# transferia/transferia

Measured on NVIDIA H100. Metric: ChangeItems/sec on ClickBench-shaped 99-col batches (filter_rows + cast + ClickHouse native block + LZ4 frames), higher is better.
Workload: dtype u8

## Files before the change

transferia_b200/csrc/kernels_encode.cuh:

```cuda
#pragma once
#include "device_types.cuh"

namespace tfk {

__device__ __forceinline__ uint32_t warp_incl_scan(uint32_t v) {
    const unsigned lane = threadIdx.x & 31;
#pragma unroll
    for (int d = 1; d < 32; d <<= 1) { uint32_t t = __shfl_up_sync(0xffffffffu, v, d); if (lane >= (unsigned)d) v += t; }
    return v;
}
__device__ __forceinline__ uint32_t block_excl_scan(uint32_t v, uint32_t* total, uint32_t* smem33) {
    const unsigned lane = threadIdx.x & 31, warp = threadIdx.x >> 5, nw = (blockDim.x + 31) >> 5;
    uint32_t inc = warp_incl_scan(v);
    if (lane == 31) smem33[warp] = inc;
    __syncthreads();
    if (warp == 0) {
        uint32_t w = lane < nw ? smem33[lane] : 0;
        uint32_t wi = warp_incl_scan(w);
        smem33[lane] = wi - w;
        if (lane == 31) smem33[32] = wi;
    }
    __syncthreads();
    uint32_t res = inc - v + smem33[warp];
    *total = smem33[32];
    __syncthreads();
    return res;
}

struct StrictCol { const uint8_t* src; uint8_t* dst; const uint8_t* validity; int32_t src_tf, dst_tf, col, pad; };
struct StrictArgs { const StrictCol* cols; int ncols; uint64_t nrows; uint8_t* err; uint16_t* term; };
__device__ __forceinline__ int64_t go_f2i64(double f) { return (f >= -9223372036854775808.0 && f < 9223372036854775808.0) ? (int64_t)f : INT64_MIN; }
__device__ __forceinline__ uint64_t go_f2u64(double f) { return f < 9223372036854775808.0 ? (uint64_t)go_f2i64(f) : ((uint64_t)go_f2i64(f - 9223372036854775808.0) ^ 0x8000000000000000ull); }
__global__ void k_strictify(StrictArgs a);
#ifdef TF_KERNELS_ENCODE
__global__ void __launch_bounds__(256) k_strictify(StrictArgs a) {
    const uint64_t r = (uint64_t)blockIdx.x * blockDim.x + threadIdx.x;
    if (r >= a.nrows) return;
    int err = 0, term = 0xff;
    for (int k = 0; k < a.ncols; k++) {
        const StrictCol c = a.cols[k];
        if (c.validity && !((c.validity[r >> 3] >> (r & 7)) & 1)) continue;
        int cls; int64_t si = 0; uint64_t ui = 0; double f = 0;
        switch (c.src_tf) {
        case TF_INT8: cls = 0; si = ((const int8_t*)c.src)[r]; break;
        case TF_INT16: cls = 0; si = ((const int16_t*)c.src)[r]; break;
        case TF_INT32: cls = 0; si = ((const int32_t*)c.src)[r]; break;
        case TF_INT64: cls = 0; si = ((const int64_t*)c.src)[r]; break;
        case TF_UINT8: cls = 1; ui = c.src[r]; break;
        case TF_UINT16: cls = 1; ui = ((const uint16_t*)c.src)[r]; break;
        case TF_UINT32: cls = 1; ui = ((const uint32_t*)c.src)[r]; break;
        case TF_UINT64: cls = 1; ui = ((const uint64_t*)c.src)[r]; break;
        case TF_FLOAT: cls = 2; f = ((const float*)c.src)[r]; break;
        case TF_DOUBLE: cls = 2; f = ((const double*)c.src)[r]; break;
        default: cls = 3; si = c.src[r] ? 1 : 0; break;
        }
        int e = 0;
        const int64_t as_i = cls == 0 || cls == 3 ? si : (cls == 1 ? (int64_t)ui : go_f2i64(f));
        const bool neg = cls == 0 ? si < 0 : (cls == 2 ? f < 0 : false);
        const uint64_t as_u = cls == 0 || cls == 3 ? (uint64_t)si : (cls == 1 ? ui : go_f2u64(f));
        auto sint = [&](int64_t lo, int64_t hi) { if (as_i < lo || as_i > hi) e = TF_ROWERR_STRICT_RANGE; };
        auto uint_ = [&](uint64_t hi) { if (neg) e = TF_ROWERR_STRICT_CAST; else if (as_u > hi) e = TF_ROWERR_STRICT_RANGE; };
        switch (c.dst_tf) {
        case TF_INT8: sint(INT8_MIN, INT8_MAX); ((int8_t*)c.dst)[r] = (int8_t)as_i; break;
        case TF_INT16: sint(INT16_MIN, INT16_MAX); ((int16_t*)c.dst)[r] = (int16_t)as_i; break;
        case TF_INT32: sint(INT32_MIN, INT32_MAX); ((int32_t*)c.dst)[r] = (int32_t)as_i; break;
        case TF_INT64: case TF_INTERVAL: case TF_DATE: case TF_DATETIME: case TF_TIMESTAMP:
            ((int64_t*)c.dst)[r] = as_i; break;
        case TF_UINT8: uint_(UINT8_MAX); c.dst[r] = (uint8_t)as_u; break;
        case TF_UINT16: uint_(UINT16_MAX); ((uint16_t*)c.dst)[r] = (uint16_t)as_u; break;
        case TF_UINT32: uint_(UINT32_MAX); ((uint32_t*)c.dst)[r] = (uint32_t)as_u; break;
        case TF_UINT64: uint_(UINT64_MAX); ((uint64_t*)c.dst)[r] = as_u; break;
        case TF_FLOAT: ((float*)c.dst)[r] = cls == 0 || cls == 3 ? (float)si : (cls == 1 ? (float)ui : (float)f); break;
        case TF_DOUBLE: ((double*)c.dst)[r] = cls == 0 ? (double)si : (cls == 1 ? (double)ui : f); break;
        default: c.dst[r] = cls == 2 ? (f != 0) : (cls == 1 ? ui != 0 : si != 0); break;
        }
        if (e && !err) { err = e; term = c.col; }
    }
    const bool mine = err && !a.err[r];
    if (mine) a.err[r] = (uint8_t)err;
    a.term[r] = (uint16_t)(mine ? term : 0xff);
}
#endif

struct RowVal {
    int cls;
    int64_t i; double f; const uint8_t* s; uint32_t slen; uint32_t nsec;
};

__device__ __forceinline__ bool row_valid(const DCol& c, uint64_t r) { return !c.validity || ((c.validity[r >> 3] >> (r & 7)) & 1); }

__device__ __forceinline__ RowVal load_val(const DCol& c, uint64_t r) {
    RowVal v; v.cls = 0; v.i = 0; v.f = 0; v.s = nullptr; v.slen = 0; v.nsec = 0;
    if (!row_valid(c, r)) return v;
    switch (c.type) {
    case TF_INT8:  v.cls = 1; v.i = ((const int8_t*)c.values)[r]; break;
    case TF_INT16: v.cls = 1; v.i = ((const int16_t*)c.values)[r]; break;
    case TF_INT32: v.cls = 1; v.i = ((const int32_t*)c.values)[r]; break;
    case TF_INT64: v.cls = 1; v.i = ((const int64_t*)c.values)[r]; break;
    case TF_UINT8:  v.cls = 1; v.i = ((const uint8_t*)c.values)[r]; break;
    case TF_UINT16: v.cls = 1; v.i = ((const uint16_t*)c.values)[r]; break;
    case TF_UINT32: v.cls = 1; v.i = ((const uint32_t*)c.values)[r]; break;
    case TF_UINT64: { uint64_t u = ((const uint64_t*)c.values)[r]; if (u > 0x7fffffffffffffffULL) v.cls = 8; else { v.cls = 1; v.i = (int64_t)u; } break; }
    case TF_FLOAT:  v.cls = 2; v.f = ((const float*)c.values)[r]; break;
    case TF_DOUBLE: v.cls = 2; v.f = ((const double*)c.values)[r]; break;
    case TF_BOOLEAN: v.cls = 3; v.i = c.values[r] != 0; v.f = v.i ? 1.0 : 0.0; break;
    case TF_INTERVAL: v.cls = 7; break;
    case TF_DATE: case TF_DATETIME: case TF_TIMESTAMP:
        v.cls = 6; v.i = ((const int64_t*)c.values)[r]; v.nsec = c.aux ? ((const uint32_t*)c.aux)[r] : 0; break;
    case TF_BYTES: v.cls = 5; v.s = c.heap + c.offsets[r]; v.slen = c.offsets[r + 1] - c.offsets[r]; break;
    case TF_UTF8:  v.cls = 4; v.s = c.heap + c.offsets[r]; v.slen = c.offsets[r + 1] - c.offsets[r]; break;
    case TF_ANY:
        if (c.aux && c.aux[r] == 1) { v.cls = 4; v.s = c.heap + c.offsets[r]; v.slen = c.offsets[r + 1] - c.offsets[r]; }
        else v.cls = 7;
        break;
    }
    return v;
}

template <typename T> __device__ __forceinline__ bool ordered(T a, T b, int op) {
    switch (op) { case 0: return a == b; case 1: return a != b; case 2: return a < b; case 3: return a <= b; case 4: return a > b; default: return a >= b; }
}
__device__ __forceinline__ int cmp_bytes(const uint8_t* a, uint32_t an, const uint8_t* b, uint32_t bn) {
    uint32_t m = an < bn ? an : bn;
    for (uint32_t k = 0; k < m; k++) { int d = (int)a[k] - (int)b[k]; if (d) return d < 0 ? -1 : 1; }
    return an < bn ? -1 : (an > bn ? 1 : 0);
}
__device__ __forceinline__ bool contains_bytes(const uint8_t* h, uint32_t hn, const uint8_t* n, uint32_t nn) {
    if (nn == 0) return true;
    if (nn > hn) return false;
    const uint8_t n0 = n[0];
    for (uint32_t i = 0; i + nn <= hn; i++) {
        if (h[i] != n0) continue;
        uint32_t k = 1; while (k < nn && h[i + k] == n[k]) k++;
        if (k == nn) return true;
    }
    return false;
}

static __device__ int eval_term(const RowVal& v, const DTerm& t, const uint8_t* blob, bool& matched) {
    const int op = t.op; const bool is_set = (op == 6 || op == 7);
    const int base = t.vtype & 15; const bool is_list = (t.vtype & 16) != 0;
    if (v.cls == 8) return TF_ROWERR_FILTER_OVERFLOW;
    if (op >= 8 && base != 4) return TF_ROWERR_FILTER_TYPEPAIR;
    const bool is_int1 = v.cls == 1;
    const bool is_float1 = v.cls == 2 || v.cls == 3 || v.cls == 0;
    const double float1 = v.cls == 2 ? v.f : (v.cls == 3 ? v.f : 0.0);
    const int64_t* il = (const int64_t*)(blob + t.list_off);
    const double* fl = (const double*)(blob + t.list_off);
    switch (base) {
    case 1:
        if (is_int1) {
            if (is_set) { bool c = false; for (int k = 0; k < t.nlist; k++) c |= (il[k] == v.i); matched = (op == 6) ? c : !c; return 0; }
            matched = ordered<int64_t>(v.i, t.i, op); return 0;
// ... 134 lines not shown
}
#endif

__global__ void k_compact_sel(const uint8_t* keep, const uint32_t* blockoff, uint64_t nrows, uint32_t* sel);
#ifdef TF_KERNELS_ENCODE
__global__ void __launch_bounds__(256) k_compact_sel(const uint8_t* keep, const uint32_t* blockoff, uint64_t nrows, uint32_t* sel) {
    __shared__ uint32_t sm[33];
    const uint64_t r = (uint64_t)blockIdx.x * blockDim.x + threadIdx.x;
    const uint32_t k = (r < nrows && keep[r]) ? 1u : 0u;
    uint32_t tot; const uint32_t ex = block_excl_scan(k, &tot, sm);
    if (k) sel[blockoff[blockIdx.x] + ex] = (uint32_t)r;
}
#endif

struct LayoutArgs {
    DCol* cols; int ncols;
    const int32_t* out_cols;
    const int32_t* str_cols; int nstr;
    const uint32_t* tile_sum;
    uint64_t* tile_base;
    uint32_t ntiles_cap;
    const uint8_t* col_headers; const uint32_t* col_header_off;
    uint8_t* raw; DState* st;
    uint64_t nrows_in; int has_sel; uint32_t frame_bytes;
    uint64_t* col_bytes;
};

#define TF_STR_TILE 256
#define TF_STR_THREADS 256
#define TF_STR_STAGE 16384

__global__ void k_layout_scan(LayoutArgs a);
#ifdef TF_KERNELS_ENCODE
__global__ void __launch_bounds__(1024) k_layout_scan(LayoutArgs a) {
    __shared__ uint32_t sm[33];
    const int s = blockIdx.x;
    const uint64_t n = a.st->n_kept;
    const uint32_t ntiles = (uint32_t)((n + TF_STR_TILE - 1) / TF_STR_TILE);
    uint64_t carry = 0;
    for (uint32_t base = 0; base < ntiles; base += blockDim.x) {
        const uint32_t i = base + threadIdx.x;
        const uint32_t v = i < ntiles ? a.tile_sum[(size_t)s * a.ntiles_cap + i] : 0;
        uint32_t tot; const uint32_t ex = block_excl_scan(v, &tot, sm);
        if (i < ntiles) a.tile_base[(size_t)s * a.ntiles_cap + i] = carry + ex;
        carry += tot;
    }
    if (threadIdx.x == 0) a.col_bytes[s] = carry;
}
#endif

__global__ void k_layout_finish(LayoutArgs a);
#ifdef TF_KERNELS_ENCODE
__global__ void __launch_bounds__(256) k_layout_finish(LayoutArgs a) {
    __shared__ uint64_t s_size[3][256];
    __shared__ uint64_t s_pos[256];
    __shared__ uint64_t s_run;
    const uint64_t n = a.st->n_kept;
    if (threadIdx.x == 0) {
        uint8_t* o = a.raw; uint64_t p = 0;
        o[p++] = 1; o[p++] = 0; o[p++] = 2; o[p++] = 0xff; o[p++] = 0xff; o[p++] = 0xff; o[p++] = 0xff; o[p++] = 0;
        uint64_t v = (uint64_t)a.ncols; while (v >= 0x80) { o[p++] = (uint8_t)(v | 0x80); v >>= 7; } o[p++] = (uint8_t)v;
        v = n; while (v >= 0x80) { o[p++] = (uint8_t)(v | 0x80); v >>= 7; } o[p++] = (uint8_t)v;
        s_run = p;
    }
    for (int base = 0; base < a.ncols; base += 256) {
        const int c = base + threadIdx.x;
        __syncthreads();
        if (c < a.ncols) {
            const DCol& d = a.cols[a.out_cols[c]];
            s_size[0][threadIdx.x] = a.col_header_off[c + 1] - a.col_header_off[c];
            s_size[1][threadIdx.x] = (d.nullable && n) ? n : 0;
            s_size[2][threadIdx.x] = n ? ((d.out_kind == OK_STR || d.out_kind == OK_TOSTR) ? a.col_bytes[d.str_slot] : (uint64_t)d.out_w * n) : 0;
        }
        __syncthreads();
        if (threadIdx.x == 0) {
            uint64_t p = s_run; const int m = a.ncols - base < 256 ? a.ncols - base : 256;
            for (int k = 0; k < m; k++) { s_pos[k] = p; p += s_size[0][k] + s_size[1][k] + s_size[2][k]; }
            s_run = p;
        }
        __syncthreads();
        if (c < a.ncols) {
            DCol& d = a.cols[a.out_cols[c]];
            const uint64_t p = s_pos[threadIdx.x];
            d.hdr_off = p; d.null_off = p + s_size[0][threadIdx.x]; d.out_off = d.null_off + s_size[1][threadIdx.x];
            const uint32_t hb = a.col_header_off[c], hn = (uint32_t)s_size[0][threadIdx.x];
            for (uint32_t k = 0; k < hn; k++) a.raw[p + k] = a.col_headers[hb + k];
        }
    }
    __syncthreads();
    if (threadIdx.x == 0) {
        const uint64_t p = s_run;
        a.st->raw_total = p;
        a.st->n_frames = p ? (p + a.frame_bytes - 1) / a.frame_bytes : 1;
        a.st->frame_ticket = 0;
    }
}
#endif

struct ColRegions { uint64_t values, validity, aux, offsets, heap, heap_len; };

__global__ void k_layout_columnar(LayoutArgs a, ColRegions* regions);
#ifdef TF_KERNELS_ENCODE
__global__ void __launch_bounds__(256) k_layout_columnar(LayoutArgs a, ColRegions* regions) {
    __shared__ uint64_t s_sz[5][256];
    __shared__ uint64_t s_pos[256];
    __shared__ uint64_t s_run;
    const uint64_t n = a.st->n_kept;
    if (threadIdx.x == 0) s_run = 0;
    for (int base = 0; base < a.ncols; base += 256) {
        const int k = base + threadIdx.x;
        __syncthreads();
        if (k < a.ncols) {
            const DCol& d = a.cols[a.out_cols[k]];
            const bool var = d.out_kind == OK_STR || d.out_kind == OK_MASK || d.out_kind == OK_TOSTR;
            const bool fresh = d.out_kind == OK_MASK || d.out_kind == OK_TOSTR || d.out_kind == OK_TODT;
            const uint64_t heap = (d.out_kind == OK_STR || d.out_kind == OK_TOSTR) ? a.col_bytes[d.str_slot] : (d.out_kind == OK_MASK ? 64 * n : 0);
            s_sz[0][threadIdx.x] = var ? 0 : (uint64_t)d.out_w * n;
            s_sz[1][threadIdx.x] = (d.validity && !fresh) ? (n + 7) / 8 : 0;
            s_sz[2][threadIdx.x] = (d.aux && !fresh) ? (d.type == TF_ANY ? n : 4 * n) : 0;
            s_sz[3][threadIdx.x] = var ? 4 * (n + 1) : 0;
            s_sz[4][threadIdx.x] = heap;
        }
        __syncthreads();
        if (threadIdx.x == 0) {
            uint64_t p = s_run; const int m = a.ncols - base < 256 ? a.ncols - base : 256;
            for (int q = 0; q < m; q++) { s_pos[q] = p; for (int z = 0; z < 5; z++) p += (s_sz[z][q] + 15) & ~15ull; }
            s_run = p;
        }
        __syncthreads();
        if (k < a.ncols) {
            DCol& d = a.cols[a.out_cols[k]];
            uint64_t p = s_pos[threadIdx.x]; ColRegions r;
            auto take = [&](int z) { const uint64_t at = p; p += (s_sz[z][threadIdx.x] + 15) & ~15ull; return at; };
            const uint64_t v = take(0), val = take(1), ax = take(2), of = take(3), hp = take(4);
            const bool var = d.out_kind == OK_STR || d.out_kind == OK_MASK || d.out_kind == OK_TOSTR;
            d.out_off = var ? hp : v; d.null_off = val; d.aux_off = ax; d.offs_off = of;
            r.values = var ? ~0ull : v; r.validity = s_sz[1][threadIdx.x] ? val : ~0ull; r.aux = s_sz[2][threadIdx.x] ? ax : ~0ull;
            r.offsets = var ? of : ~0ull; r.heap = var ? hp : ~0ull; r.heap_len = s_sz[4][threadIdx.x];
            regions[k] = r;
            if (var) ((uint32_t*)(a.raw + of))[n] = (uint32_t)s_sz[4][threadIdx.x];
        }
    }
    __syncthreads();
    if (threadIdx.x == 0) { a.st->raw_total = s_run; a.st->n_frames = 0; a.st->frame_ticket = 0; }
}
#endif

struct EncodeArgs {
    const DCol* cols;
    const int32_t* slots;
    const uint32_t* sel; const DState* st; uint8_t* raw;
    uint32_t* tile_sum; const uint64_t* tile_base; uint32_t ntiles_cap;
    int columnar;
};

#define TF_SLOT_NULLMAP (1 << 30)
#define TF_SLOT_AUX (1 << 29)
#define TF_SLOT_ZEROMAP (1 << 28)
#define TF_FIX_TILE_WORDS 2048
#define CH_MAX_DATE_SEC 4291747200LL

enum StreamKind { SK_COPY = 0, SK_BOOL, SK_DATE, SK_DATETIME, SK_TS64, SK_NULLMAP, SK_AUX32, SK_AUX8, SK_ZERO, SK_TODT_CH, SK_TODT_SEC };

template <int K, int INW> __device__ __forceinline__ uint64_t elem_t(const DCol& c, const uint32_t* sel, uint64_t j, uint64_t n) {
    if (j >= n) return 0;
    const uint64_t r = sel ? sel[j] : j;
    if (K == SK_ZERO) return 0;
    if (K == SK_TODT_CH || K == SK_TODT_SEC) {
        int64_t s = 0;
        if (row_valid(c, r)) s = c.type == TF_INT32 ? (int64_t)((const int32_t*)c.values)[r] : (int64_t)((const uint32_t*)c.values)[r];
        if (K == SK_TODT_SEC) return (uint64_t)s;
        if (s > CH_MAX_DATE_SEC) s = CH_MAX_DATE_SEC;
        if (s < 0) s = 0;
        return (uint64_t)s;
    }
    if (K == SK_AUX8) return (uint64_t)c.aux[r];
    if (K == SK_AUX32) return (uint64_t)((const uint32_t*)c.aux)[r];
    const bool valid = row_valid(c, r);
    if (K == SK_NULLMAP) return valid ? 0 : 1;
    if (!valid) return 0;
    if (K == SK_COPY) {
        if (INW == 1) return c.values[r];
        if (INW == 2) return ((const uint16_t*)c.values)[r];
        if (INW == 4) return ((const uint32_t*)c.values)[r];
        return ((const uint64_t*)c.values)[r];
    }
    if (K == SK_BOOL) return c.values[r] != 0;
    if (K == SK_DATE || K == SK_DATETIME) {
        int64_t s = ((const int64_t*)c.values)[r];
        const uint32_t ns = c.aux ? ((const uint32_t*)c.aux)[r] : 0;
        if (s > CH_MAX_DATE_SEC || (s == CH_MAX_DATE_SEC && ns > 0)) s = CH_MAX_DATE_SEC;
        if (s < 0) s = 0;
        return K == SK_DATE ? (uint64_t)(s / 86400) : (uint64_t)s;
    }
    const int64_t s = ((const int64_t*)c.values)[r];
    const uint32_t ns = c.aux ? ((const uint32_t*)c.aux)[r] : 0;
    return (uint64_t)(s * 1000000LL + (int64_t)(ns / 1000u));
}

template <int K, int INW, int W> __device__ __forceinline__ uint32_t stream_word_t(const DCol& c, const uint32_t* sel, uint64_t q, uint64_t n) {
    if (W == 1) return (uint32_t)elem_t<K, INW>(c, sel, 4 * q, n) | ((uint32_t)elem_t<K, INW>(c, sel, 4 * q + 1, n) << 8) |
                       ((uint32_t)elem_t<K, INW>(c, sel, 4 * q + 2, n) << 16) | ((uint32_t)elem_t<K, INW>(c, sel, 4 * q + 3, n) << 24);
    if (W == 2) return (uint32_t)(elem_t<K, INW>(c, sel, 2 * q, n) & 0xffff) | ((uint32_t)(elem_t<K, INW>(c, sel, 2 * q + 1, n) & 0xffff) << 16);
    if (W == 4) return (uint32_t)elem_t<K, INW>(c, sel, q, n);
    const uint64_t v = elem_t<K, INW>(c, sel, q >> 1, n); return (uint32_t)(v >> ((q & 1) * 32));
}

template <int K, int INW, int W> __device__ __forceinline__ void encode_stream(const DCol& c, const EncodeArgs& a, uint64_t base, uint64_t n) {
    const uint32_t m = (uint32_t)(base & 3);
    const uint64_t total = n * (uint64_t)W;
    const uint64_t T = (m + total + 3) >> 2;
    uint8_t* dst0 = a.raw + (base - m);
    const unsigned lane = threadIdx.x & 31;
    for (uint64_t t0 = (uint64_t)blockIdx.x * TF_FIX_TILE_WORDS; t0 < T; t0 += (uint64_t)gridDim.x * TF_FIX_TILE_WORDS)
#pragma unroll 2
    for (uint32_t it = 0; it < TF_FIX_TILE_WORDS / 256; it++) {
        const uint64_t t = t0 + it * 256 + threadIdx.x;
        const uint32_t wcur = (t < T) ? stream_word_t<K, INW, W>(c, a.sel, t, n) : 0;
        uint32_t wprev = __shfl_up_sync(0xffffffffu, wcur, 1);
        if (lane == 0) wprev = (m && t > 0 && t <= T) ? stream_word_t<K, INW, W>(c, a.sel, t - 1, n) : 0;
        if (t >= T) continue;
        const uint32_t val = m ? __funnelshift_r(wprev, wcur, 8 * (4 - m)) : wcur;
        const int64_t sb = (int64_t)(4 * t) - (int64_t)m;
        uint8_t* dst = dst0 + 4 * t;
        if (sb >= 0 && (uint64_t)sb + 4 <= total) *(uint32_t*)dst = val;
        else {
#pragma unroll
            for (int b = 0; b < 4; b++) { const int64_t x = sb + b; if (x >= 0 && (uint64_t)x < total) dst[b] = (uint8_t)(val >> (8 * b)); }
        }
    }
}

__global__ void k_encode_fixed(EncodeArgs a);
#ifdef TF_KERNELS_ENCODE
__global__ void __launch_bounds__(256) k_encode_fixed(EncodeArgs a) {
    const int32_t slot = a.slots[blockIdx.y];
    const DCol c = a.cols[slot & ~(TF_SLOT_NULLMAP | TF_SLOT_AUX | TF_SLOT_ZEROMAP)];
    const uint64_t n = a.st->n_kept;
    if (n == 0) return;
    const DCol& cc = c;
    if (slot & TF_SLOT_ZEROMAP) { encode_stream<SK_ZERO, 1, 1>(cc, a, c.null_off, n); return; }
    if (slot & TF_SLOT_NULLMAP) { encode_stream<SK_NULLMAP, 1, 1>(c, a, c.null_off, n); return; }
    if (slot & TF_SLOT_AUX) { if (c.type == TF_ANY) encode_stream<SK_AUX8, 1, 1>(c, a, c.aux_off, n); else encode_stream<SK_AUX32, 4, 4>(c, a, c.aux_off, n); return; }
    switch (c.out_kind) {
    case OK_COPY:
        switch (c.in_w) {
        case 1: encode_stream<SK_COPY, 1, 1>(c, a, c.out_off, n); break;
        case 2: encode_stream<SK_COPY, 2, 2>(c, a, c.out_off, n); break;
        case 4: encode_stream<SK_COPY, 4, 4>(c, a, c.out_off, n); break;
        default: encode_stream<SK_COPY, 8, 8>(c, a, c.out_off, n); break;
        }
        break;
    case OK_BOOL: encode_stream<SK_BOOL, 1, 1>(c, a, c.out_off, n); break;
    case OK_DATE: encode_stream<SK_DATE, 8, 2>(c, a, c.out_off, n); break;
    case OK_DATETIME: encode_stream<SK_DATETIME, 8, 4>(c, a, c.out_off, n); break;
    case OK_TS64: encode_stream<SK_TS64, 8, 8>(c, a, c.out_off, n); break;
    case OK_TODT: if (a.columnar) encode_stream<SK_TODT_SEC, 4, 8>(c, a, c.out_off, n); else encode_stream<SK_TODT_CH, 4, 4>(c, a, c.out_off, n); break;
    }
}
#endif

__global__ void k_pack_validity(EncodeArgs a);
#ifdef TF_KERNELS_ENCODE
__global__ void __launch_bounds__(256) k_pack_validity(EncodeArgs a) {
    const DCol c = a.cols[a.slots[blockIdx.y]];
    const uint64_t n = a.st->n_kept;
    const uint64_t b = (uint64_t)blockIdx.x * blockDim.x + threadIdx.x;
    if (b * 8 >= n) return;
    uint32_t v = 0;
#pragma unroll
    for (int k = 0; k < 8; k++) {
        const uint64_t j = b * 8 + k;
        if (j < n) { const uint64_t r = a.sel ? a.sel[j] : j; v |= (row_valid(c, r) ? 1u : 0u) << k; }
    }
    a.raw[c.null_off + b] = (uint8_t)v;
}
#endif


struct MeasureArgs { const DCol* cols; int ncols; uint64_t nrows; uint64_t* per_row; unsigned long long* total; };

__global__ void k_measure(MeasureArgs a);
#ifdef TF_KERNELS_ENCODE
__global__ void __launch_bounds__(256) k_measure(MeasureArgs a) {
    __shared__ uint32_t sm[33];
    const uint64_t r = (uint64_t)blockIdx.x * blockDim.x + threadIdx.x;
    uint64_t sz = 0;
    if (r < a.nrows) {
        sz = 24;
        for (int c = 0; c < a.ncols; c++) {
            const DCol& d = a.cols[c];
            sz += 16;
            if (!row_valid(d, r)) continue;
            switch (d.type) {
            case TF_UTF8: sz += 16 + (d.offsets[r + 1] - d.offsets[r]); break;
            case TF_ANY: sz += 16 + (d.offsets[r + 1] - d.offsets[r]); break;
            case TF_BYTES: sz += 24 + (d.offsets[r + 1] - d.offsets[r]); break;
            case TF_DATE: case TF_DATETIME: case TF_TIMESTAMP: sz += 24; break;
            default: sz += (uint64_t)d.in_w;
            }
        }
        if (a.per_row) a.per_row[r] = sz;
    }
    const uint32_t lo = (uint32_t)(sz & 0xffffffu), hi = (uint32_t)(sz >> 24);
    uint32_t tl, th; block_excl_scan(lo, &tl, sm); __syncthreads(); block_excl_scan(hi, &th, sm);
    if (threadIdx.x == 0) atomicAdd(a.total, (unsigned long long)tl + ((unsigned long long)th << 24));
}
#endif

}
```

transferia_b200/csrc/tfgpu.cu:

```cuda
#include <cuda_runtime.h>
#include <algorithm>
#include <chrono>
#include <cstdio>
#include <cstdlib>
#include <cstring>
#include <memory>
#include <string>
#include <vector>

#include "../../include/tfgpu.h"
#include "../../include/tfgpu_sink.h"
#include "plan.hpp"
#include "device_types.cuh"
#include "launch.hpp"
#include "host_internal.hpp"

using namespace tfk;

namespace {

#define CK(x) do { cudaError_t _e = (x); if (_e != cudaSuccess) throw CudaError{_e, #x}; } while (0)

inline size_t align_up(size_t v, size_t a) { return (v + a - 1) / a * a; }

// ... 276 lines not shown
DCol make_dcol(const tf_col& ic, int type) {
    DCol d; std::memset(&d, 0, sizeof d);
    d.type = type; d.in_w = in_width(type); d.str_slot = -1; d.mask_slot = -1;
    d.values = (const uint8_t*)ic.values; d.validity = ic.validity; d.offsets = ic.offsets; d.heap = ic.heap; d.aux = (const uint8_t*)ic.aux;
    return d;
}

void ensure_d_cols(tfgpu_engine* e, size_t nc) {
    if (e->d_cols_cap >= nc) return;
    if (e->d_cols) CK(cudaFree(e->d_cols));
    CK(cudaMalloc(&e->d_cols, sizeof(DCol) * nc)); e->d_cols_cap = nc;
}

uint32_t grid_cap(const tfgpu_engine* e, uint32_t tiles_upper, uint32_t nslots, uint32_t waves) {
    const uint32_t want = ((uint32_t)e->sm_count * 6u * waves + nslots - 1) / (nslots ? nslots : 1);
    return std::max(1u, std::min(tiles_upper, std::max(want, 8u)));
}

void run_deflate(tfgpu_engine* e, const uint8_t* text, uint64_t total, bool zlib) {
    cudaStream_t s = e->stream;
    const uint64_t nch = (total + DF_CHUNK - 1) / DF_CHUNK;
    if (nch >= (1ull << 32)) throw tfplan::FatalError(TF_E_FATAL_ARG, "row text too large to compress in one call");
    e->wire.ensure(total + nch * DF_CHUNK_OVERHEAD + 64);
    Layout L;
    const size_t o_pfx = L.take(nch * 8), o_sums = L.take(nch * 8), o_ticket = L.take(4);
    e->defl_meta.ensure(L.total());
    uint8_t* M = e->defl_meta.p;
    CK(cudaMemsetAsync(M + o_pfx, 0, nch * 8, s)); CK(cudaMemsetAsync(M + o_ticket, 0, 4, s));
    DeflateArgs da{text, total, e->wire.p, (unsigned long long*)(M + o_pfx), (uint32_t*)(M + o_sums), (uint32_t*)(M + o_ticket), (uint32_t)nch, zlib ? 1 : 0, e->d_state};
    if (nch) {
        const uint32_t grid = (uint32_t)std::min<uint64_t>(nch, (uint64_t)e->sm_count * 2);
        TF_LAUNCH(e, k_deflate_chunks, grid, DF_THREADS, df_smem().total, s, da);
    }
    TF_LAUNCH(e, k_deflate_finish, 1, 1024, 0, s, da);
}

void run_zstd(tfgpu_engine* e, const uint8_t* text, uint64_t total) {
    cudaStream_t s = e->stream;
    const uint64_t nch = (total + ZS_CHUNK - 1) / ZS_CHUNK;
    if (nch >= (1ull << 32)) throw tfplan::FatalError(TF_E_FATAL_ARG, "row text too large to compress in one call");
    e->wire.ensure(total + nch * 3 + 64);
    Layout L;
    const size_t o_pfx = L.take(nch * 8), o_ticket = L.take(4);
    e->zstd_meta.ensure(L.total());
    uint8_t* M = e->zstd_meta.p;
    CK(cudaMemsetAsync(M + o_pfx, 0, nch * 8, s)); CK(cudaMemsetAsync(M + o_ticket, 0, 4, s));
    ZstdArgs za{text, total, e->wire.p, (unsigned long long*)(M + o_pfx), (uint32_t*)(M + o_ticket), (uint32_t)nch, e->d_state};
    if (nch) {
        const uint32_t grid = (uint32_t)std::min<uint64_t>(nch, (uint64_t)e->sm_count);
        TF_LAUNCH(e, k_zstd_chunks, grid, ZS_THREADS, zs_smem().total, s, za);
    }
    TF_LAUNCH(e, k_zstd_finish, 1, 32, 0, s, za);
}

struct ChainOut { uint8_t* errcode; uint16_t* errstep; const uint32_t* sel; bool has_sharder; };

ChainOut run_chain(tfgpu_engine* e, PlanDev& pd, uint64_t n, const tf_col* dev_cols, const uint8_t* dev_kinds, int out_fmt, const uint8_t* pre_err = nullptr, const DbzEmitArgs* dz = nullptr) {
    const bool columnar = out_fmt == 0;
    const tfplan::Plan& pl = pd.plan;
    const size_t nc = pl.in_schema.size();
    const int wire_base = out_fmt & 0xff;
    const bool dbz = wire_base == TF_WIRE_DEBEZIUM;
    const bool ser = wire_base == TF_WIRE_SER_JSON || wire_base == TF_WIRE_SER_CSV || dbz;
    const bool json_rows = wire_base == TF_WIRE_CH_JSONEACHROW || ser;
    if (ser) for (size_t c = 0; c < nc; c++) if (pd.col_out_kind[c] == OK_TOSTR && pl.in_schema[c].tf == TF_ANY)
        throw tfplan::FatalError(TF_E_FATAL_UNSUPPORTED, "serializer sinks after convert_to_string on an `any` column are not handled on the device");
    const Sizes sz = compute_sizes(e, pd, n, dev_cols, columnar, json_rows);
    cudaStream_t s = e->stream;
    if (e->tail_pending && !(out_fmt == TF_WIRE_CH_NATIVE_LZ4 && n == e->tail_nrows && (const void*)&pd == e->tail_plan && sz.n_frames_max == e->tail_nframes_max)) join_tail(e);
    const size_t nslot_alloc = (size_t)(pd.n_str > 0 ? pd.n_str : 1);
    Layout W;
    const size_t o_keep = W.take(n), o_errcode = W.take(n), o_errstep = W.take(2 * n), o_blockcnt = W.take(sz.nblocks * 4), o_blockoff = W.take(sz.nblocks * 4),
                 o_sel = W.take(n * 4), o_tile_sum = W.take(nslot_alloc * sz.ntiles_cap * 4), o_tile_base = W.take(nslot_alloc * sz.ntiles_cap * 8),
                 o_comp = W.take(sz.n_frames_max * 4), o_wire_off = W.take(sz.n_frames_max * 8), o_pfx = W.take(sz.n_frames_max * 8), o_col_bytes = W.take(nslot_alloc * 8);
    e->work.ensure(W.total());
    uint8_t* w = e->work.p;
    uint8_t* keep = w + o_keep; uint8_t* errcode = w + o_errcode; uint16_t* errstep = (uint16_t*)(w + o_errstep); uint32_t* blockcnt = (uint32_t*)(w + o_blockcnt); uint32_t* blockoff = (uint32_t*)(w + o_blockoff);
    uint32_t* tile_sum = (uint32_t*)(w + o_tile_sum); uint64_t* tile_base = (uint64_t*)(w + o_tile_base); uint64_t* col_bytes = (uint64_t*)(w + o_col_bytes);
    uint32_t* comp_size = (uint32_t*)(w + o_comp); uint64_t* wire_off = (uint64_t*)(w + o_wire_off); unsigned long long* frame_pfx = (unsigned long long*)(w + o_pfx);
    e->raw.ensure(sz.raw_bound);
    const bool lz = out_fmt == TF_WIRE_CH_NATIVE_LZ4;
    if (lz) e->wire.ensure(sz.wire_bound);
    ensure_d_cols(e, nc);
    std::vector<DCol> hc(nc); std::vector<StrictCol> strict;
    for (size_t c = 0; c < nc; c++) {
        const tf_col& ic = dev_cols[c];
        int ctype = ic.type;
        if (ic.type != pl.in_schema[c].tf) {
            const int st = ic.type, dt = pl.in_schema[c].tf;
            const bool s_num = in_width(st) && st != TF_INTERVAL && st != TF_DATE && st != TF_DATETIME && st != TF_TIMESTAMP;
            if ((st == TF_UTF8 && dt == TF_BYTES) || (st == TF_BYTES && dt == TF_UTF8)) ctype = dt;
            else if (s_num && in_width(dt) && !(st == TF_FLOAT && dt == TF_DOUBLE) && !(st == TF_BOOLEAN && dt == TF_DOUBLE)) { strict.push_back(StrictCol{(const uint8_t*)ic.values, nullptr, ic.validity, st, dt, (int32_t)c, 0}); ctype = dt; }
            else throw tfplan::FatalError(TF_E_FATAL_ARG, "column " + std::to_string(c) + ": a " + std::to_string(st) + " value cannot be strictified to the plan's column type on the device");
        }
        DCol& d = hc[c]; d = make_dcol(ic, ctype);
        d.out_kind = pd.col_out_kind[c]; d.out_w = pd.col_out_w[c];
        if (columnar && d.out_kind == OK_TODT) d.out_w = 8;
        else if (columnar && d.out_kind != OK_STR && d.out_kind != OK_MASK && d.out_kind != OK_TOSTR) { d.out_kind = OK_COPY; d.out_w = d.in_w; }
        d.nullable = pd.col_nullable[c]; d.str_slot = pd.col_str_slot[c]; d.mask_slot = pd.col_mask_slot[c];
        if (n) {
            if (d.in_w && !d.values) throw tfplan::FatalError(TF_E_FATAL_ARG, "column " + std::to_string(c) + ": values pointer is NULL");
            if (!d.in_w && !d.offsets) throw tfplan::FatalError(TF_E_FATAL_ARG, "column " + std::to_string(c) + ": offsets pointer is NULL");
        }
    }
    const uint16_t* pre_term = nullptr;
    if (!strict.empty() && n) {
        Layout S;
        const size_t o_desc = S.take(strict.size() * sizeof(StrictCol)), o_err = S.take(n), o_term = S.take(2 * n);
        std::vector<size_t> o_val(strict.size());
        for (size_t k = 0; k < strict.size(); k++) o_val[k] = S.take((size_t)in_width(strict[k].dst_tf) * n + 16);
        e->strict_stage.ensure(S.total() + 256);
        uint8_t* B = e->strict_stage.p;
        for (size_t k = 0; k < strict.size(); k++) { strict[k].dst = B + o_val[k]; hc[strict[k].col].values = B + o_val[k]; }
        CK(cudaMemcpyAsync(B + o_desc, strict.data(), strict.size() * sizeof(StrictCol), cudaMemcpyHostToDevice, s));
        if (pre_err) CK(cudaMemcpyAsync(B + o_err, pre_err, n, cudaMemcpyDeviceToDevice, s)); else CK(cudaMemsetAsync(B + o_err, 0, n, s));
        StrictArgs sa{(const StrictCol*)(B + o_desc), (int)strict.size(), n, B + o_err, (uint16_t*)(B + o_term)};
        TF_LAUNCH(e, k_strictify, (uint32_t)((n + 255) / 256), 256, 0, s, sa);
        pre_err = B + o_err; pre_term = (const uint16_t*)(B + o_term);
    }
    CK(cudaMemcpyAsync(e->d_cols, hc.data(), sizeof(DCol) * nc, cudaMemcpyHostToDevice, s));
    CK(cudaMemsetAsync(e->d_state, 0, sizeof(DState), s));
    if (!pl.n2f_cols.empty() && n) {
        const size_t k2 = pl.n2f_cols.size();
        Layout S;
        const size_t o_which = S.take(k2 * 4), o_len = S.take(k2 * n * 4), o_off = S.take(k2 * (n + 1) * 4), o_tot = S.take(k2 * 8 + 8), o_base = S.take(k2 * 8 + 8), o_err = S.take(n);
        e->n2f_stage.ensure(S.total() + 256);
        uint8_t* B = e->n2f_stage.p;
        std::vector<int32_t> which(pl.n2f_cols.begin(), pl.n2f_cols.end());
        CK(cudaMemcpyAsync(B + o_which, which.data(), k2 * 4, cudaMemcpyHostToDevice, s));
        if (pre_err) CK(cudaMemcpyAsync(B + o_err, pre_err, n, cudaMemcpyDeviceToDevice, s)); else CK(cudaMemsetAsync(B + o_err, 0, n, s));
        N2fArgs na{e->d_cols, (const int32_t*)(B + o_which), dev_kinds, n, (uint32_t*)(B + o_len), (const uint32_t*)(B + o_off), nullptr, (const uint64_t*)(B + o_base), B + o_err};
        TF_LAUNCH(e, k_n2f_sizes, dim3((uint32_t)((n + 127) / 128), (uint32_t)k2), 128, 0, s, na);
        const Heaps h = size_heaps(e, (const uint32_t*)(B + o_len), n, (uint32_t)k2, (uint32_t*)(B + o_off), (uint64_t*)(B + o_tot), (uint64_t*)(B + o_base),
                                   e->n2f_heap, "number_to_float: a rewritten column exceeds 4 GiB");
        na.heap = e->n2f_heap.p;
        TF_LAUNCH(e, k_n2f_write, dim3((uint32_t)((n + 127) / 128), (uint32_t)k2), 128, 0, s, na);
        for (size_t k = 0; k < k2; k++) { DCol& d = hc[pl.n2f_cols[k]]; d.offsets = (const uint32_t*)(B + o_off) + k * (n + 1); d.heap = e->n2f_heap.p + h.base[k]; }
        CK(cudaMemcpyAsync(e->d_cols, hc.data(), sizeof(DCol) * nc, cudaMemcpyHostToDevice, s));
        pre_err = B + o_err;
    }
    const bool sink_guard = dev_kinds && !columnar && !dbz;
    const bool has_filter = pd.n_fsteps > 0 || pre_err || sink_guard;
    e->last_wire_fmt = out_fmt;
    const uint32_t nb = (uint32_t)((n + 255) / 256);
    uint32_t* sel = (has_filter && n) ? (uint32_t*)(w + o_sel) : nullptr;
    if (sel) {
        FilterArgs fa{e->d_cols, dev_kinds, n, pd.d_fsteps, pd.n_fsteps, pd.d_expr_off, pd.d_terms, pd.d_blob, keep, errcode, errstep, blockcnt, e->d_state, pre_err, pre_term, sink_guard ? 1 : 0};
        TF_LAUNCH(e, k_filter, nb, 256, 0, s, fa);
        TF_LAUNCH(e, k_scan_blockcnt, 1, 1024, 0, s, blockcnt, blockoff, nb, e->d_state);
        TF_LAUNCH(e, k_compact_sel, nb, 256, 0, s, keep, blockoff, n, sel);
    }
    const uint32_t ntiles = (uint32_t)((n + TF_STR_TILE - 1) / TF_STR_TILE);
    const uint32_t str_gx = std::max(1u, (ntiles + TF_STR_GROUP - 1) / TF_STR_GROUP);
    EncodeArgs ea{e->d_cols, pd.d_str_slots, sel, e->d_state, e->raw.p, tile_sum, tile_base, sz.ntiles_cap, columnar ? 1 : 0};
    if (!has_filter || !n) {
        DState init; std::memset(&init, 0, sizeof init); init.n_kept = n;
        CK(cudaMemcpyAsync(e->d_state, &init, sizeof init, cudaMemcpyHostToDevice, s));
    }
    if (pl.has_sharder && n) {
        e->part_ids.ensure(n * 4 + 256);
        ShardArgs sa{e->d_cols, pd.d_shard_cols, (int)pl.shard_cols.size(), pd.d_mask_keys, sel, e->d_state, pl.shards, (uint32_t*)e->part_ids.p};
        TF_LAUNCH(e, k_shard_ids, nb, 256, 0, s, sa);
    }
    if (json_rows) {
        const uint32_t jt = (uint32_t)((n + TF_JSON_TILE - 1) / TF_JSON_TILE);
        JsonArgs ja{e->d_cols, ser ? (wire_base == TF_WIRE_SER_CSV ? pd.d_scsvcols : pd.d_sjcols) : pd.d_jcols, (int)pl.out_cols.size(), ser ? pd.d_snames : pd.d_jnames, pd.d_mask_keys, sel, e->d_state, e->raw.p,
                    (uint32_t*)e->work_json_sizes(n), tile_sum, tile_base, col_bytes,
                    dbz ? 3 : ser ? (wire_base == TF_WIRE_SER_JSON ? 1 : 2) : 0, (uint32_t)(((out_fmt & TF_WIRE_F_CLOSING_NEWLINE) ? TF_SER_NL : 0) | ((out_fmt & TF_WIRE_F_ANY_AS_STRING) ? TF_SER_AAS : 0)), errcode, errstep, DbzEmitArgs{}};
        if (dbz) { ja.jcols = pd.d_sjcols; e->dbz_keysz.ensure(n * 4 + 256); e->dbz_msgsz.ensure(n * 28 + 256); ja.dz = *dz; ja.dz.key_size = (uint32_t*)e->dbz_keysz.p; ja.dz.msg_size = (uint32_t*)e->dbz_msgsz.p; }
        if (ser && !has_filter && n) { CK(cudaMemsetAsync(errcode, 0, n, s)); CK(cudaMemsetAsync(errstep, 0, 2 * n, s)); }
        if (jt) TF_LAUNCH(e, k_json_sizes, jt, TF_JSON_TILE, 0, s, ja);
        LayoutArgs lj{e->d_cols, 0, pd.d_out_cols, pd.d_str_slots, 1, tile_sum, tile_base, sz.ntiles_cap, pd.d_col_headers, pd.d_col_header_off,
                      e->raw.p, e->d_state, n, 1, e->frame_bytes, col_bytes};
        TF_LAUNCH(e, k_layout_scan, 1, 1024, 0, s, lj);
        uint64_t json_total = 0;
        {
            CK(cudaMemcpyAsync(&json_total, col_bytes, 8, cudaMemcpyDeviceToHost, s)); CK(cudaStreamSynchronize(s));
            e->raw.ensure(json_total + 256); ja.raw = e->raw.p;
        }
        TF_LAUNCH(e, k_json_write, jt ? jt : 1, TF_JSON_TILE, 0, s, ja);
        if (ser && (out_fmt & (TF_WIRE_F_GZIP | TF_WIRE_F_ZLIB))) run_deflate(e, e->raw.p, n ? json_total : 0, (out_fmt & TF_WIRE_F_ZLIB) != 0);
        if (out_fmt & TF_WIRE_F_ZSTD) run_zstd(e, e->raw.p, n ? json_total : 0);
        return ChainOut{errcode, errstep, sel, pl.has_sharder};
    }
    if (pd.n_str && ntiles) TF_LAUNCH(e, k_str_sizes, dim3(str_gx, pd.n_str), TF_STR_THREADS, 0, s, ea);
    LayoutArgs la{e->d_cols, (int)pl.out_cols.size(), pd.d_out_cols, pd.d_str_slots, pd.n_str, tile_sum, tile_base, sz.ntiles_cap, pd.d_col_headers, pd.d_col_header_off,
                  e->raw.p, e->d_state, n, 1, e->frame_bytes, col_bytes};
    if (pd.n_str) TF_LAUNCH(e, k_layout_scan, pd.n_str, 1024, 0, s, la);
    const int32_t* fixed_slots = pd.d_fixed_slots; uint32_t n_fixed = (uint32_t)pd.n_fixed_slots, n_valid = 0;
    if (!columnar) TF_LAUNCH(e, k_layout_finish, 1, 256, 0, s, la);
    else {
        const size_t no = pl.out_cols.size();
        if (e->d_call_cap < no) {
            if (e->d_call_slots) { CK(cudaFree(e->d_call_slots)); CK(cudaFree(e->d_regions)); }
            CK(cudaMalloc(&e->d_call_slots, sizeof(int32_t) * 3 * no)); CK(cudaMalloc(&e->d_regions, sizeof(ColRegions) * no)); e->d_call_cap = no;
        }
        std::vector<int32_t> fixed, valid;
        for (int oc : pl.out_cols) {
            const DCol& d = hc[oc];
            if (d.out_kind == OK_COPY || d.out_kind == OK_TODT) fixed.push_back(oc);
            const bool fresh = d.out_kind == OK_MASK || d.out_kind == OK_TOSTR || d.out_kind == OK_TODT;
            if (!fresh && d.aux) fixed.push_back(oc | TF_SLOT_AUX);
            if (!fresh && d.validity) valid.push_back(oc);
        }
        fixed_slots = e->d_call_slots; n_fixed = (uint32_t)fixed.size(); n_valid = (uint32_t)valid.size();
        fixed.insert(fixed.end(), valid.begin(), valid.end());
        if (!fixed.empty()) CK(cudaMemcpyAsync(e->d_call_slots, fixed.data(), fixed.size() * 4, cudaMemcpyHostToDevice, s));
        TF_LAUNCH(e, k_layout_columnar, 1, 256, 0, s, la, e->d_regions);
    }
    if (n) {
        if (n_fixed) {
            const uint32_t gx = grid_cap(e, (uint32_t)((2 * n + 2 + TF_FIX_TILE_WORDS - 1) / TF_FIX_TILE_WORDS), n_fixed, 6);
            EncodeArgs fa = ea; fa.slots = fixed_slots;
            TF_LAUNCH(e, k_encode_fixed, dim3(gx, n_fixed), 256, 0, s, fa);
        }
        if (n_valid) {
            EncodeArgs va = ea; va.slots = fixed_slots + n_fixed;
            TF_LAUNCH(e, k_pack_validity, dim3((uint32_t)((n / 8 + 256) / 256), n_valid), 256, 0, s, va);
        }
        if (pd.n_str) TF_LAUNCH(e, k_encode_str_plain, dim3(str_gx, pd.n_str), TF_STR_THREADS, 0, s, ea);
        if (pd.n_str && pd.n_tostr) TF_LAUNCH(e, k_encode_str, dim3(ntiles, pd.n_str), TF_STR_THREADS, 0, s, ea);
        if (pd.n_mask_cols) {
            MaskArgs ma{e->d_cols, pd.d_mask_slots, pd.d_mask_keys, sel, e->d_state, e->raw.p, columnar ? 1 : 0};
            TF_LAUNCH(e, k_mask_encode, dim3((uint32_t)((n + 127) / 128), pd.n_mask_cols), 128, 0, s, ma);
        }
    }
    if (lz) {
        Lz4Args za{e->raw.p, e->d_state, e->wire.p, comp_size, wire_off, frame_pfx, e->d_tail, e->frame_bytes, e->lz_phases};
        const size_t smem = lz_smem(e->frame_bytes).total;
        const uint32_t per_sm = (uint32_t)std::max<size_t>(1, std::min<size_t>(LZ_CTAS_PER_SM, (227 * 1024) / (smem + 1024)));
        const uint32_t grid = (uint32_t)std::min<uint64_t>(sz.n_frames_max, (uint64_t)e->sm_count * per_sm);
        join_tail(e);
        CK(cudaMemsetAsync(frame_pfx, 0, sz.n_frames_max * 8, s));
        TF_LAUNCH(e, k_lz4_frames, grid, LZ_THREADS, smem, s, za);
        FrameArgs fa{comp_size, wire_off, e->wire.p, e->d_tail};
        cudaStream_t s3 = e->side_stream;
        CK(cudaEventRecord(e->ev_fork, s)); CK(cudaStreamWaitEvent(s3, e->ev_fork, 0));
        TF_LAUNCH(e, k_frame_seal, (uint32_t)((sz.n_frames_max + 31) / 32), 32, SEAL_SMEM, s3, fa);
        CK(cudaEventRecord(e->ev_tail, s3));
        e->tail_pending = true; e->tail_nrows = n; e->tail_plan = (const void*)&pd; e->tail_nframes_max = sz.n_frames_max;
    }
    return ChainOut{errcode, errstep, sel, pl.has_sharder};
}

}


static bool wire_is_ser(int wire_fmt) {
    const int b = wire_fmt & 0xff;
    return (b == TF_WIRE_SER_JSON || b == TF_WIRE_SER_CSV) && (wire_fmt & ~(0xff | TF_WIRE_F_CLOSING_NEWLINE | TF_WIRE_F_ANY_AS_STRING | TF_WIRE_F_GZIP | TF_WIRE_F_ZLIB)) == 0 &&
           (wire_fmt & (TF_WIRE_F_GZIP | TF_WIRE_F_ZLIB)) != (TF_WIRE_F_GZIP | TF_WIRE_F_ZLIB);
}
static bool wire_known(int wire_fmt) {
    return wire_fmt == TF_WIRE_CH_NATIVE || wire_fmt == TF_WIRE_CH_NATIVE_LZ4 || wire_fmt == TF_WIRE_CH_JSONEACHROW ||
           wire_fmt == (TF_WIRE_CH_JSONEACHROW | TF_WIRE_F_ZSTD) || wire_is_ser(wire_fmt);
}

static int check_batch(tfgpu_engine* e, int plan_id, const tf_batch* in, PlanDev*& pd) {
    if (!e || !in || plan_id < 0 || plan_id >= (int)e->plans.size()) return TF_E_FATAL_ARG;
    pd = e->plans[plan_id].get();
    if (in->ncols != pd->plan.in_schema.size()) return fail(e, TF_E_FATAL_ARG, "batch column count does not match the plan schema");
    if (in->nrows >= (1ull << 31)) return fail(e, TF_E_FATAL_ARG, "batch too large (>= 2^31 rows)");
    return TF_OK;
}

extern "C" {

const char* tfgpu_version(void) { return "tfgpu 0.1.0 sm_90a"; }

int tfgpu_engine_create(const char* cfg_json, const int* device_ids, int n_devices, tfgpu_engine** out) {
    if (!out) return TF_E_FATAL_ARG;
    *out = nullptr;
    int ndev = 0;
    if (cudaGetDeviceCount(&ndev) != cudaSuccess || ndev == 0) { cudaGetLastError(); return TF_E_FATAL_NODEVICE; }
    if (n_devices > 1) return TF_E_FATAL_ARG;
    auto e = std::make_unique<tfgpu_engine>();
    e->device = (n_devices == 1 && device_ids) ? device_ids[0] : 0;
    if (e->device < 0 || e->device >= ndev) return TF_E_FATAL_ARG;
    try {
        if (cfg_json && *cfg_json) {
            auto cfg = tfj::parse(cfg_json);
            double fb = cfg->get_num("frame_bytes", LZ_MAX_FRAME);
            if (fb < 1024 || fb > LZ_MAX_FRAME || ((uint32_t)fb & 15)) return TF_E_FATAL_CONFIG;
            e->frame_bytes = (uint32_t)fb;
        }
        CK(cudaSetDevice(e->device));
        cudaDeviceProp prop; CK(cudaGetDeviceProperties(&prop, e->device));
        e->sm_count = prop.multiProcessorCount;
        CK(cudaStreamCreateWithFlags(&e->own_stream, cudaStreamNonBlocking));
        e->stream = e->own_stream;
        CK(cudaStreamCreateWithFlags(&e->side_stream, cudaStreamNonBlocking));
        CK(cudaEventCreateWithFlags(&e->ev_tail, cudaEventDisableTiming));
        CK(cudaMalloc(&e->d_tail, 64)); CK(cudaMemset(e->d_tail, 0, 64));
        CK(cudaEventCreateWithFlags(&e->ev_fork, cudaEventDisableTiming));
        CK(cudaMalloc(&e->d_state, sizeof(DState)));
        const struct { const void* k; size_t smem; } big_smem[] = {
            {(const void*)k_lz4_frames, lz_smem(LZ_MAX_FRAME).total}, {(const void*)k_frame_seal, SEAL_SMEM},
            {(const void*)k_dbz_pass1, DBZ_STAGE}, {(const void*)k_deflate_chunks, df_smem().total}, {(const void*)k_zstd_chunks, zs_smem().total}};
        for (const auto& b : big_smem) CK(cudaFuncSetAttribute(b.k, cudaFuncAttributeMaxDynamicSharedMemorySize, (int)b.smem));
    } catch (const CudaError& c) { return c.e == cudaErrorMemoryAllocation ? TF_E_RETRY_OOM : TF_E_RETRY_LAUNCH; }
    catch (const std::exception&) { return TF_E_FATAL_CONFIG; }
    *out = e.release();
    return TF_OK;
}

int tfgpu_engine_destroy(tfgpu_engine* e) {
    if (!e) return TF_E_FATAL_ARG;
// ... 1029 lines not shown
```

Before: 1.150 billion.

## Encode fixed-width columns by scanning source rows with in-tile compaction

Instead of gathering each kept row through the selection index, the fixed-width encoder walks source rows in tiles, reads them coalesced (with 16-byte vector loads for aligned plain copy columns), and compacts kept values in shared memory through ballot/scan before writing each tile's output run. A selectivity heuristic picks between this row-scan path and the existing gather-stream path. It adds shared-memory staging, extra syncs and a launch_bounds occupancy hint, and relies on the filter's keep flags and per-block offsets lining up with the tile boundaries.

```diff
diff --git a/transferia_b200/csrc/kernels_encode.cuh b/transferia_b200/csrc/kernels_encode.cuh
--- a/transferia_b200/csrc/kernels_encode.cuh
+++ b/transferia_b200/csrc/kernels_encode.cuh
@@ -1,4 +1,5 @@
 #pragma once
+#include <type_traits>
 #include "device_types.cuh"
 
 namespace tfk {
@@ -439,6 +440,7 @@
     const uint32_t* sel; const DState* st; uint8_t* raw;
     uint32_t* tile_sum; const uint64_t* tile_base; uint32_t ntiles_cap;
     int columnar;
+    const uint8_t* keep; const uint32_t* blockoff; uint64_t nrows;
 };
 
 #define TF_SLOT_NULLMAP (1 << 30)
@@ -518,31 +520,175 @@
     }
 }
 
+#define TF_FIX_ROW_TILE 1024
+struct FixStage {
+    uint64_t run[TF_FIX_ROW_TILE + 2];
+    uint32_t off[TF_FIX_ROW_TILE / 32 + 1];
+};
+__device__ __forceinline__ void write_run(const EncodeArgs& a, const FixStage& sm, uint64_t at, int32_t len) {
+    const uint32_t* const pw = (const uint32_t*)(sm.run + 1);
+    const int32_t m = (int32_t)(at & 3);
+    uint8_t* const dst0 = a.raw + (at - m);
+    for (int32_t w = threadIdx.x; 4 * w < m + len; w += blockDim.x) {
+        const uint32_t hi = pw[w], val = m ? __funnelshift_r(pw[w - 1], hi, 8 * (4 - m)) : hi;
+        const int32_t sb = 4 * w - m;
+        uint8_t* dst = dst0 + 4 * w;
+        if (sb >= 0 && sb + 4 <= len) *(uint32_t*)dst = val;
+        else {
+#pragma unroll
+            for (int b = 0; b < 4; b++) if (sb + b >= 0 && sb + b < len) dst[b] = (uint8_t)(val >> (8 * b));
+        }
+    }
+}
+template <int K, int INW, int W> __device__ __forceinline__ void encode_rows(const DCol& c, const EncodeArgs& a, uint64_t base, FixStage& sm) {
+    typedef typename std::conditional<W == 1, uint8_t, typename std::conditional<W == 2, uint16_t,
+            typename std::conditional<W == 4, uint32_t, uint64_t>::type>::type>::type T;
+    constexpr int KB = TF_FIX_ROW_TILE / 256, ROWS = TF_FIX_ROW_TILE, NC = 8 * KB;
+    static_assert(NC == 32, "one warp scans the tile's counts");
+    const unsigned lane = threadIdx.x & 31, warp = threadIdx.x >> 5;
+    T* const packed = (T*)(sm.run + 1);
+    const uint32_t nrows = (uint32_t)a.nrows, nt = (nrows + ROWS - 1) / ROWS;
+    for (uint32_t t = blockIdx.x; t < nt; t += gridDim.x) {
+        const uint32_t r0 = t * ROWS;
+        T v[KB]; unsigned kept = 0;
+#pragma unroll
+        for (int k = 0; k < KB; k++) {
+            const uint32_t r = r0 + 256 * k + threadIdx.x;
+            if (r < nrows && (!a.sel || a.keep[r])) kept |= 1u << k;
+            v[k] = (T)elem_t<K, INW>(c, nullptr, r, nrows);
+        }
+#pragma unroll
+        for (int k = 0; k < KB; k++) {
+            const unsigned b = __ballot_sync(0xffffffffu, (kept >> k) & 1);
+            if (lane == 0) sm.off[k * 8 + warp] = __popc(b);
+        }
+        __syncthreads();
+        if (warp == 0) {
+            const uint32_t c = sm.off[lane], inc = warp_incl_scan(c);
+            sm.off[lane] = inc - c;
+            if (lane == 31) sm.off[NC] = inc;
+        }
+        __syncthreads();
+#pragma unroll
+        for (int k = 0; k < KB; k++) {
+            const unsigned b = __ballot_sync(0xffffffffu, (kept >> k) & 1);
+            if ((kept >> k) & 1) packed[sm.off[k * 8 + warp] + __popc(b & ((1u << lane) - 1u))] = v[k];
+        }
+        __syncthreads();
+        write_run(a, sm, base + (uint64_t)(a.sel ? a.blockoff[t * KB] : r0) * W, (int32_t)sm.off[NC] * W);
+        __syncthreads();
+    }
+}
+
+__device__ __forceinline__ uint32_t& vec_word(uint4& v, int k) { return k == 0 ? v.x : k == 1 ? v.y : k == 2 ? v.z : v.w; }
+template <int INW> __device__ __forceinline__ void encode_rows_vec(const DCol& c, const EncodeArgs& a, uint64_t base, FixStage& sm) {
+    typedef typename std::conditional<INW == 1, uint8_t, typename std::conditional<INW == 2, uint16_t,
+            typename std::conditional<INW == 4, uint32_t, uint64_t>::type>::type>::type T;
+    constexpr int R = 16 / INW, U = 2, ROWS = 256 * U * R, NC = 8 * U;
+    static_assert(ROWS * INW <= 8 * TF_FIX_ROW_TILE, "tile larger than its stage");
+    const unsigned lane = threadIdx.x & 31, warp = threadIdx.x >> 5;
+    T* const packed = (T*)(sm.run + 1);
+    const uint32_t nrows = (uint32_t)a.nrows, nt = (nrows + ROWS - 1) / ROWS;
+    for (uint32_t t = blockIdx.x; t < nt; t += gridDim.x) {
+        const uint32_t r0 = t * ROWS;
+        uint4 v[U]; uint32_t kept = 0;
+#pragma unroll
+        for (int u = 0; u < U; u++) {
+            const uint32_t r = r0 + (u * 256 + threadIdx.x) * R;
+            v[u] = make_uint4(0, 0, 0, 0);
+            if (r + R <= nrows) {
+                v[u] = *(const uint4*)(c.values + (uint64_t)r * INW);
+                uint32_t kb = (1u << R) - 1u;
+                if (a.sel) {
+                    const uint8_t* kp = a.keep + r;
+                    uint32_t f[4] = {0, 0, 0, 0};
+                    if (R == 16) { const uint4 q = *(const uint4*)kp; f[0] = q.x; f[1] = q.y; f[2] = q.z; f[3] = q.w; }
+                    else if (R == 8) { const uint2 q = *(const uint2*)kp; f[0] = q.x; f[1] = q.y; }
+                    else if (R == 4) f[0] = *(const uint32_t*)kp;
+                    else f[0] = *(const uint16_t*)kp;
+                    kb = 0;
+#pragma unroll
+                    for (int i = 0; i < R; i++) kb |= ((f[i >> 2] >> (8 * (i & 3))) & 0xffu ? 1u : 0u) << i;
+                }
+                kept |= kb << (u * R);
+            } else {
+#pragma unroll
+                for (int i = 0; i < R; i++) {
+                    if (r + i < nrows && (!a.sel || a.keep[r + i])) {
+                        kept |= 1u << (u * R + i);
+                        const uint64_t x = ((const T*)c.values)[r + i];
+                        if (INW == 8) { if (i == 0) { v[u].x = (uint32_t)x; v[u].y = (uint32_t)(x >> 32); } else { v[u].z = (uint32_t)x; v[u].w = (uint32_t)(x >> 32); } }
+                        else vec_word(v[u], i * INW / 4) |= (uint32_t)x << (8 * (i * INW % 4));
+                    }
+                }
+            }
+        }
+        uint32_t incl[U];
+#pragma unroll
+        for (int u = 0; u < U; u++) {
+            const uint32_t cnt = __popc((kept >> (u * R)) & ((1u << R) - 1u));
+            incl[u] = warp_incl_scan(cnt);
+            if (lane == 31) sm.off[u * 8 + warp] = incl[u];
+            incl[u] -= cnt;
+        }
+        __syncthreads();
+        if (warp == 0) {
+            const uint32_t cw = lane < NC ? sm.off[lane] : 0, inc = warp_incl_scan(cw);
+            if (lane < NC) sm.off[lane] = inc - cw;
+            if (lane == 31) sm.off[TF_FIX_ROW_TILE / 32] = inc;
+        }
+        __syncthreads();
+#pragma unroll
+        for (int u = 0; u < U; u++) {
+            uint32_t pos = sm.off[u * 8 + warp] + incl[u];
+#pragma unroll
+            for (int i = 0; i < R; i++)
+                if ((kept >> (u * R + i)) & 1)
+                    packed[pos++] = INW == 8 ? (T)(i == 0 ? ((uint64_t)v[u].y << 32 | v[u].x) : ((uint64_t)v[u].w << 32 | v[u].z))
+                                             : (T)(vec_word(v[u], i * INW / 4) >> (8 * (i * INW % 4)));
+        }
+        __syncthreads();
+        write_run(a, sm, base + (uint64_t)(a.sel ? a.blockoff[r0 / 256] : r0) * INW, (int32_t)sm.off[TF_FIX_ROW_TILE / 32] * INW);
+        __syncthreads();
+    }
+}
+
+#define TF_FIX_ROWS_MIN_SECTORS 0.5f
+
+template <int K, int INW, int W> __device__ __forceinline__ void encode_any(const DCol& c, const EncodeArgs& a, uint64_t base, uint64_t n, FixStage& sm) {
+    const float rows_per_sector = K == SK_NULLMAP ? 256.f : 32.f / INW;
+    const bool rows = K != SK_ZERO &&
+                      (!a.sel || 1.f - powf(1.f - (float)n / (float)a.nrows, rows_per_sector) > TF_FIX_ROWS_MIN_SECTORS);
+    if (rows && K == SK_COPY && !c.validity && ((uintptr_t)c.values & 15) == 0) encode_rows_vec<INW>(c, a, base, sm);
+    else if (rows) encode_rows<K, INW, W>(c, a, base, sm);
+    else encode_stream<K, INW, W>(c, a, base, n);
+}
+
 __global__ void k_encode_fixed(EncodeArgs a);
 #ifdef TF_KERNELS_ENCODE
-__global__ void __launch_bounds__(256) k_encode_fixed(EncodeArgs a) {
+__global__ void __launch_bounds__(256, 6) k_encode_fixed(EncodeArgs a) {
+    __shared__ FixStage sm;
     const int32_t slot = a.slots[blockIdx.y];
     const DCol c = a.cols[slot & ~(TF_SLOT_NULLMAP | TF_SLOT_AUX | TF_SLOT_ZEROMAP)];
     const uint64_t n = a.st->n_kept;
     if (n == 0) return;
-    const DCol& cc = c;
-    if (slot & TF_SLOT_ZEROMAP) { encode_stream<SK_ZERO, 1, 1>(cc, a, c.null_off, n); return; }
-    if (slot & TF_SLOT_NULLMAP) { encode_stream<SK_NULLMAP, 1, 1>(c, a, c.null_off, n); return; }
-    if (slot & TF_SLOT_AUX) { if (c.type == TF_ANY) encode_stream<SK_AUX8, 1, 1>(c, a, c.aux_off, n); else encode_stream<SK_AUX32, 4, 4>(c, a, c.aux_off, n); return; }
+    if (slot & TF_SLOT_ZEROMAP) { encode_any<SK_ZERO, 1, 1>(c, a, c.null_off, n, sm); return; }
+    if (slot & TF_SLOT_NULLMAP) { encode_any<SK_NULLMAP, 1, 1>(c, a, c.null_off, n, sm); return; }
+    if (slot & TF_SLOT_AUX) { if (c.type == TF_ANY) encode_any<SK_AUX8, 1, 1>(c, a, c.aux_off, n, sm); else encode_any<SK_AUX32, 4, 4>(c, a, c.aux_off, n, sm); return; }
     switch (c.out_kind) {
     case OK_COPY:
         switch (c.in_w) {
-        case 1: encode_stream<SK_COPY, 1, 1>(c, a, c.out_off, n); break;
-        case 2: encode_stream<SK_COPY, 2, 2>(c, a, c.out_off, n); break;
-        case 4: encode_stream<SK_COPY, 4, 4>(c, a, c.out_off, n); break;
-        default: encode_stream<SK_COPY, 8, 8>(c, a, c.out_off, n); break;
+        case 1: encode_any<SK_COPY, 1, 1>(c, a, c.out_off, n, sm); break;
+        case 2: encode_any<SK_COPY, 2, 2>(c, a, c.out_off, n, sm); break;
+        case 4: encode_any<SK_COPY, 4, 4>(c, a, c.out_off, n, sm); break;
+        default: encode_any<SK_COPY, 8, 8>(c, a, c.out_off, n, sm); break;
         }
         break;
-    case OK_BOOL: encode_stream<SK_BOOL, 1, 1>(c, a, c.out_off, n); break;
-    case OK_DATE: encode_stream<SK_DATE, 8, 2>(c, a, c.out_off, n); break;
-    case OK_DATETIME: encode_stream<SK_DATETIME, 8, 4>(c, a, c.out_off, n); break;
-    case OK_TS64: encode_stream<SK_TS64, 8, 8>(c, a, c.out_off, n); break;
-    case OK_TODT: if (a.columnar) encode_stream<SK_TODT_SEC, 4, 8>(c, a, c.out_off, n); else encode_stream<SK_TODT_CH, 4, 4>(c, a, c.out_off, n); break;
+    case OK_BOOL: encode_any<SK_BOOL, 1, 1>(c, a, c.out_off, n, sm); break;
+    case OK_DATE: encode_any<SK_DATE, 8, 2>(c, a, c.out_off, n, sm); break;
+    case OK_DATETIME: encode_any<SK_DATETIME, 8, 4>(c, a, c.out_off, n, sm); break;
+    case OK_TS64: encode_any<SK_TS64, 8, 8>(c, a, c.out_off, n, sm); break;
+    case OK_TODT: if (a.columnar) encode_any<SK_TODT_SEC, 4, 8>(c, a, c.out_off, n, sm); else encode_any<SK_TODT_CH, 4, 4>(c, a, c.out_off, n, sm); break;
     }
 }
 #endif
diff --git a/transferia_b200/csrc/tfgpu.cu b/transferia_b200/csrc/tfgpu.cu
--- a/transferia_b200/csrc/tfgpu.cu
+++ b/transferia_b200/csrc/tfgpu.cu
@@ -452,7 +452,7 @@
     }
     const uint32_t ntiles = (uint32_t)((n + TF_STR_TILE - 1) / TF_STR_TILE);
     const uint32_t str_gx = std::max(1u, (ntiles + TF_STR_GROUP - 1) / TF_STR_GROUP);
-    EncodeArgs ea{e->d_cols, pd.d_str_slots, sel, e->d_state, e->raw.p, tile_sum, tile_base, sz.ntiles_cap, columnar ? 1 : 0};
+    EncodeArgs ea{e->d_cols, pd.d_str_slots, sel, e->d_state, e->raw.p, tile_sum, tile_base, sz.ntiles_cap, columnar ? 1 : 0, keep, blockoff, n};
     if (!has_filter || !n) {
         DState init; std::memset(&init, 0, sizeof init); init.n_kept = n;
         CK(cudaMemcpyAsync(e->d_state, &init, sizeof init, cudaMemcpyHostToDevice, s));
```

Measured after the change: 1.168 billion (median of 6 runs). 1.02x the previous value.
